# mungerct/Stabilized_Navier_Stokes_Flow_FEniCSx

Hardware: NVIDIA B200
Metric: NS Jacobian+residual assembly throughput (higher is better)
Workload: dtype f64

## Files before the change

### stabilized_navier_stokes_flow_fenicsx_b200/csrc/element_p1tet.cuh

```cuda
#pragma once
#include "element_generic.cuh"

namespace nsgpu {

#if defined(__CUDA_ARCH__)
#define NS_RSQRT(x) rsqrt(x)
#else
#define NS_RSQRT(x) (1.0 / sqrt(x))
#endif

constexpr double P1T_A = 0.1381966011250105;
constexpr double P1T_E = 0.4472135954999579;

template <bool WANT_J, bool WANT_F>
NS_HD void p1tet_rowslab(const FormParams& fp, const bool row_is_origin, const double (&x)[4][3], const double (&u)[4][3],
                         const double (&p)[4], double (&blk)[4][16], double (&fr)[4]) {
  double J[3][3];
#pragma unroll
  for (int i = 0; i < 3; ++i)
#pragma unroll
    for (int j = 0; j < 3; ++j) J[i][j] = x[j + 1][i] - x[0][i];
  const double c00 = J[1][1] * J[2][2] - J[1][2] * J[2][1];
  const double c01 = J[1][2] * J[2][0] - J[1][0] * J[2][2];
  const double c02 = J[1][0] * J[2][1] - J[1][1] * J[2][0];
// ... 229 lines not shown
      s[i] += wt * pt.uq[i];
      Y3[i] += be * pt.Gu[i];
      if (WANT_F) sup[i] += al * pt.uq[i];
    }
    {
      const double w0 = wt * pt.uq[0], w1 = wt * pt.uq[1], w2 = wt * pt.uq[2];
      Q[0] += w0 * pt.uq[0]; Q[1] += w0 * pt.uq[1]; Q[2] += w0 * pt.uq[2];
      Q[3] += w1 * pt.uq[1]; Q[4] += w1 * pt.uq[2]; Q[5] += w2 * pt.uq[2];
    }
    if (WANT_J) {
#pragma unroll
      for (int d = 0; d < 3; ++d) {
        const double bg = be * pt.Gu[d];
#pragma unroll
        for (int c = 0; c < 3; ++c) Y1[d][c] += bg * pt.uq[c];
      }
    }
    if (q == 0) {
      pt0 = pt;
#pragma unroll
      for (int d = 0; d < 3; ++d) ub[d] = W * (P1T_A * U[d] + P1T_E * pt.uq[d]);
    } else if (WANT_J) {
      scratch.put(q, pt);
    }
  }
  nuLbar *= itrG;

  const double TR0 = tbar * Pg0 + H[0] * s[0] + H[1] * s[1] + H[2] * s[2];
  scratch.get_D(D);

  if (WANT_F) {
    const double pbarV = W * (p[0] + p[1] + p[2] + p[3]);
#pragma unroll
    for (int c = 0; c < 3; ++c)
      fr[c] = D[c][0] * ub[0] + D[c][1] * ub[1] + D[c][2] * ub[2] + fp.nu * V * H[c] - pbarV * g[0][c] + sup[c] + nuLbar * divu * g[0][c];
    fr[3] = W * divu + TR0;
  }

  if (WANT_J) {
    const double kap = divu * itrG;
    const double M_off = W * (4.0 * P1T_A * P1T_A + 2.0 * P1T_A * P1T_E);
    const double akap = P1T_A * kap;
    const double ZG[3] = {G[0] * s[0] + G[1] * s[1] + G[2] * s[2], G[1] * s[0] + G[3] * s[1] + G[4] * s[2],
                          G[2] * s[0] + G[4] * s[1] + G[5] * s[2]};
    double C0[3][3], P0[3];
#pragma unroll
    for (int c = 0; c < 3; ++c)
#pragma unroll
      for (int d = 0; d < 3; ++d)
        C0[c][d] = M_off * D[c][d] + P1T_A * (s[c] * H[d] - Y1[d][c]) + akap * ZG[d] * g[0][c];
#pragma unroll
    for (int d = 0; d < 3; ++d) P0[d] = P1T_A * (tbar * H[d] - Y3[d]);
    const double dia0 = P1T_A * TR0;
    const double nuV = fp.nu * V;
    const double Qm[3][3] = {{Q[0], Q[1], Q[2]}, {Q[1], Q[3], Q[4]}, {Q[2], Q[4], Q[5]}};
#pragma unroll
    for (int n = 0; n < 4; ++n) {
      P1TetPoint pt;
      if (n == 0) pt = pt0; else { scratch.get(n, pt); scratch.get_g(n, g[n]); }
      const double L = g[0][0] * g[n][0] + g[0][1] * g[n][1] + g[0][2] * g[n][2];
      double t1[3], t2[3];
      const double ewk = pt.ew * kap;
#pragma unroll
      for (int d = 0; d < 3; ++d) {
        t1[d] = pt.ew * H[d] - pt.eb * pt.Gu[d];
        t2[d] = ewk * pt.Gu[d] + nuLbar * g[n][d];
      }
      const double dia = ub[0] * g[n][0] + ub[1] * g[n][1] + ub[2] * g[n][2] + nuV * L + dia0 + pt.ea;
      double blk[16];
#pragma unroll
      for (int c = 0; c < 3; ++c) {
#pragma unroll
        for (int d = 0; d < 3; ++d) {
          double v = C0[c][d] + L * Qm[c][d] + pt.uq[c] * t1[d] + g[0][c] * t2[d];
          if (n == 0) v += (W * P1T_E * P1T_E) * D[c][d];
          if (c == d) v += dia;
          blk[4 * c + d] = v;
        }
        blk[4 * c + 3] = s[c] * L - W * g[0][c];
      }
#pragma unroll
      for (int d = 0; d < 3; ++d) blk[12 + d] = P0[d] + W * g[n][d] + t1[d] + s[d] * L;
      blk[15] = tbar * L;
      emit(n, blk);
    }
  }
}

}
struct nsgpu_ctx;
namespace nsgpu {
bool p1tet_fast_available(nsgpu_ctx* ctx);
int p1tet_assemble(nsgpu_ctx* ctx, const double* d_xin, bool want_J, bool want_F, double* d_Fout, int part = 0, int sm_reserve = 0);
bool p1tet_can_split(nsgpu_ctx* ctx);
int p1tet_build_plan(nsgpu_ctx* ctx);
void p1tet_free(nsgpu_ctx* ctx);
void p1tet_mark_bc_dirty(nsgpu_ctx* ctx);
int p1tet_spmv(nsgpu_ctx* ctx, const double* d_x, double* d_y);
struct P1BlockView { int64_t n_ent; const int64_t* pair0; const int32_t* ns; const int64_t* rowpos; const int32_t* rowdof; };
bool p1tet_block_view(nsgpu_ctx* ctx, P1BlockView* out);
int p1tet_assemble_streamed(nsgpu_ctx* ctx, const double* x_host, double* F_host);
}
```

### stabilized_navier_stokes_flow_fenicsx_b200/csrc/p1tet.cu

```cuda
#include <algorithm>
#include <cstdio>
#include <vector>
#include <cstdlib>
#include <cub/cub.cuh>

#include "common.cuh"
#include "element_p1tet.cuh"

constexpr int TILE_MAX_ENT = 40;
constexpr int PIPE_VCAP = 128;

struct TileHdr {
  int64_t e0;
  int64_t boff;
  int nent, ninc, nslots, nv;
};

struct nsgpu_p1tet_plan {
  int64_t n_inc = 0, n_ent = 0, n_tiles = 0, n_slots = 0;
  int cap = 0, maxdeg = 0, max_nent = 0;
  uint32_t* d_inc_cell = nullptr;
  int4* d_inc_vtx = nullptr;
  int4* d_inc_lead = nullptr;
  int2* d_tile_vlist = nullptr;
// ... 252 lines not shown
        int pick = pos;
        if (want >= 0)
          for (int c = pos; c < len[l]; ++c)
            if (((base[l] + (lst[l][c] >> 2)) & 7) == want) { pick = c; break; }
        const uint8_t tmp = lst[l][pos]; lst[l][pos] = lst[l][pick]; lst[l][pick] = tmp;
      }
    }
  }
  (void)nt;
}

__global__ void __launch_bounds__(128) k_tile_vlist(TileHdr* __restrict__ hdr, const int4* __restrict__ p_vtx, const int4* __restrict__ p_lead,
                                                    int2* __restrict__ vlist, uint32_t* __restrict__ inc_loc, int* max_nv) {
  using Sort = cub::BlockRadixSort<uint32_t, 128, 4>;
  using Scan = cub::BlockScan<int, 128>;
  __shared__ union { typename Sort::TempStorage sort; typename Scan::TempStorage scan; } tmp;
  __shared__ uint32_t sorted[512], uniq[512];
  const int64_t t = blockIdx.x;
  const int tid = threadIdx.x;
  const int ninc = hdr[t].ninc;
  const int4 vt = p_vtx[t * 128 + tid], ld = p_lead[t * 128 + tid];
  const uint32_t vtx[4] = {(uint32_t)vt.x, (uint32_t)vt.y, (uint32_t)vt.z, (uint32_t)vt.w};
  const int lead[4] = {ld.x, ld.y, ld.z, ld.w};
  uint32_t keys[4];
#pragma unroll
  for (int a = 0; a < 4; ++a) keys[a] = tid < ninc ? vtx[a] : 0xffffffffu;
  Sort(tmp.sort).Sort(keys);
#pragma unroll
  for (int k = 0; k < 4; ++k) sorted[4 * tid + k] = keys[k];
  __syncthreads();
  int flags[4], pos[4], total = 0;
#pragma unroll
  for (int k = 0; k < 4; ++k) {
    const int i = 4 * tid + k;
    flags[k] = (keys[k] != 0xffffffffu && (i == 0 || sorted[i - 1] != keys[k])) ? 1 : 0;
  }
  Scan(tmp.scan).ExclusiveSum(flags, pos, total);
#pragma unroll
  for (int k = 0; k < 4; ++k)
    if (flags[k]) uniq[pos[k]] = keys[k];
  __syncthreads();
  uint32_t packed = 0;
  if (tid < ninc) {
#pragma unroll
    for (int a = 0; a < 4; ++a) {
      int lo = 0, hi = total - 1;
      while (lo < hi) {
        const int mid = (lo + hi) >> 1;
        if (uniq[mid] < vtx[a]) lo = mid + 1; else hi = mid;
      }
      if (lo < PIPE_VCAP) vlist[t * PIPE_VCAP + lo] = make_int2((int)vtx[a], lead[a]);
      packed |= (uint32_t)(lo & 255) << (8 * a);
    }
  }
  __shared__ uint32_t first_packed;
  if (tid == 0) first_packed = packed;
  __syncthreads();
  inc_loc[t * 128 + tid] = tid < ninc ? packed : first_packed;
  if (tid == 0) { hdr[t].nv = total; atomicMax(max_nv, total); }
}

constexpr uint32_t INC_BC_BIT = 0x80000000u;
__global__ void k_inc_bc(int64_t n, uint32_t* __restrict__ inc_cell, const int32_t* __restrict__ dofmap, const uint8_t* __restrict__ marker) {
  const int64_t i = blockIdx.x * (int64_t)blockDim.x + threadIdx.x;
  if (i >= n) return;
  const uint32_t cm = inc_cell[i] & ~INC_BC_BIT;
  const int64_t c = cm >> 2;
  uint8_t f = 0;
  if (marker)
    for (int k = 0; k < 16; ++k) f |= marker[dofmap[c * 16 + k]];
  inc_cell[i] = cm | (f ? INC_BC_BIT : 0u);
}

template <int CAP, int ECAP = CAP> struct TileSmem {
  static constexpr int kBytes = ((5 * CAP + 1 + 15) & ~15) + ((4 * CAP + 15) & ~15) + ((CAP + 15) & ~15);
  static constexpr size_t stageJ = 16 * (size_t)CAP * sizeof(double4);
  static constexpr size_t stageF = (size_t)CAP * sizeof(double4);
  static constexpr size_t tables = 32 * ECAP + 16 * ECAP + 8 * (ECAP + 2) + 4 * CAP + kBytes;
  static constexpr size_t bytes(bool want_J) { return (want_J ? stageJ : 0) + stageF + tables; }
};

template <int CAP_, bool WANT_J, int ECAP = CAP_> struct TileView {
  static constexpr int CAP = CAP_;
  double2* stageJ; double4* stageF; int64_t* rowpos; int4* rowdof; int2* rel; uint32_t* src; uint8_t* bytes;
  __device__ explicit TileView(unsigned char* raw) {
    stageJ = reinterpret_cast<double2*>(raw);
    stageF = reinterpret_cast<double4*>(stageJ + (WANT_J ? 32 * CAP : 0));
    rowpos = reinterpret_cast<int64_t*>(stageF + CAP);
    rowdof = reinterpret_cast<int4*>(rowpos + 4 * ECAP);
    rel = reinterpret_cast<int2*>(rowdof + ECAP);
    src = reinterpret_cast<uint32_t*>(rel + (ECAP + 2));
    bytes = reinterpret_cast<uint8_t*>(src + CAP);
  }
};

__device__ __forceinline__ void cp_async16(void* smem, const void* gmem) {
  asm volatile("cp.async.cg.shared.global [%0], [%1], 16;\n" ::"r"((unsigned)__cvta_generic_to_shared(smem)), "l"(gmem) : "memory");
}
__device__ __forceinline__ void cp_async16_ca(void* smem, const void* gmem) {
  asm volatile("cp.async.ca.shared.global [%0], [%1], 16;\n" ::"r"((unsigned)__cvta_generic_to_shared(smem)), "l"(gmem) : "memory");
}
__device__ __forceinline__ void cp_async8(void* smem, const void* gmem) {
  asm volatile("cp.async.ca.shared.global [%0], [%1], 8;\n" ::"r"((unsigned)__cvta_generic_to_shared(smem)), "l"(gmem) : "memory");
}
__device__ __forceinline__ void cp_async4(void* smem, const void* gmem) {
  asm volatile("cp.async.ca.shared.global [%0], [%1], 4;\n" ::"r"((unsigned)__cvta_generic_to_shared(smem)), "l"(gmem) : "memory");
}
__device__ __forceinline__ void cp_async_commit() { asm volatile("cp.async.commit_group;\n" ::: "memory"); }
__device__ __forceinline__ void cp_async_wait_all() { asm volatile("cp.async.wait_all;\n" ::: "memory"); }
template <int N> __device__ __forceinline__ void cp_async_wait_group() { asm volatile("cp.async.wait_group %0;\n" ::"n"(N) : "memory"); }

template <int CAP, int NT, bool WANT_J, class View>
__device__ __forceinline__ void tile_tables_async(const View& v, const TileHdr& h, int tid, int64_t tile,
                                                  const uint32_t* __restrict__ src, const uint8_t* __restrict__ tile_bytes,
                                                  const int2* __restrict__ ent_rel, const int64_t* __restrict__ rowpos,
                                                  const int4* __restrict__ rowdof) {
  if (WANT_J) {
    for (int k = tid; k < CAP / 4; k += NT) cp_async16(v.src + 4 * k, src + tile * CAP + 4 * k);
    const int nb = (pad16(h.nslots + h.nent + 1) + pad16(h.nslots) + pad16(h.nent)) >> 4;
    for (int k = tid; k < nb; k += NT) cp_async16(v.bytes + 16 * k, tile_bytes + h.boff + 16 * k);
  }
  for (int k = tid; k < h.nent; k += NT) {
    cp_async8(v.rel + k, ent_rel + h.e0 + k);
    cp_async16(v.rowdof + k, rowdof + h.e0 + k);
    if (WANT_J) {
      cp_async16(v.rowpos + 4 * k, rowpos + 4 * (h.e0 + k));
      cp_async16(v.rowpos + 4 * k + 2, rowpos + 4 * (h.e0 + k) + 2);
    }
  }
  if (tid == 0) v.rel[h.nent] = make_int2(h.ninc, h.nslots);
}

__device__ __forceinline__ double quad_sum_b(double v) {
  v += __shfl_xor_sync(0xffffffffu, v, 1);
  v += __shfl_xor_sync(0xffffffffu, v, 2);
  return v;
}

__device__ __forceinline__ int stage_idx(const int CAP, const int n, const int k, const int i) { return (n * 8 + k) * CAP + i; }

__device__ __forceinline__ void store_piece(double* dst, const double4& a, const bool wide) {
  if (wide) {
    asm volatile("st.global.cs.v4.f64 [%0], {%1, %2, %3, %4};" ::"l"(dst), "d"(a.x), "d"(a.y), "d"(a.z), "d"(a.w) : "memory");
  } else {
    __stcs(reinterpret_cast<double2*>(dst), make_double2(a.x, a.y));
    __stcs(reinterpret_cast<double2*>(dst) + 1, make_double2(a.z, a.w));
  }
}

template <int CAP, int NT, bool WANT_J, bool WANT_F, class View>
__device__ __forceinline__ void tile_gather(const View& v, const TileHdr& h, int tid, double* __restrict__ vals,
                                            double* __restrict__ F, const bool wide = false) {
  const uint8_t* s_ss = v.bytes;
  const uint8_t* eos = v.bytes + pad16(h.nslots + h.nent + 1);
  const uint8_t* dg = eos + pad16(h.nslots);
  if (WANT_J) {
    const uint8_t* srcb = reinterpret_cast<const uint8_t*>(v.src);
    for (int ls = tid; ls < h.nslots; ls += NT) {
      const int le = eos[ls];
      const int2 rel = v.rel[le];
      const int s = ls - rel.y;
      if (s == dg[le]) continue;
      const uint8_t* ss = s_ss + ls + le;
      const int jb = ss[0], je = ss[1];
      const uint8_t* sp = srcb + 4 * rel.x;
      double4 acc[4];
// ... 4 lines not shown
#pragma unroll
        for (int i = 0; i < 3; ++i) {
          const bool ok = q + i < je;
          const int code = ok ? sp[q + i] : 0;
          const double2* blkp = v.stageJ + (code & 3) * 8 * CAP + rel.x + (code >> 2);
#pragma unroll
          for (int k = 0; k < 8; ++k) t[i][k] = ok ? blkp[k * CAP] : make_double2(0.0, 0.0);
        }
#pragma unroll
        for (int r = 0; r < 4; ++r) {
          acc[r].x += (t[0][2 * r].x + t[1][2 * r].x) + t[2][2 * r].x;
          acc[r].y += (t[0][2 * r].y + t[1][2 * r].y) + t[2][2 * r].y;
          acc[r].z += (t[0][2 * r + 1].x + t[1][2 * r + 1].x) + t[2][2 * r + 1].x;
          acc[r].w += (t[0][2 * r + 1].y + t[1][2 * r + 1].y) + t[2][2 * r + 1].y;
        }
      }
#pragma unroll
      for (int r = 0; r < 4; ++r) {
        double* dst = vals + v.rowpos[4 * le + r] + 4 * s;
        store_piece(dst, acc[r], wide);
      }
    }
  }
  {
    const int nD = 16 * h.nent;
    const double* sf = reinterpret_cast<const double*>(v.stageF);
    for (int base = 0; base < nD; base += NT) {
      const int item = base + (NT - 1 - tid);
      const int part = item & 3, r = (item >> 2) & 3, le = item >> 4;
      double4 acc = make_double4(0.0, 0.0, 0.0, 0.0);
      double accF = 0.0;
      if (le < h.nent) {
        const int ib = v.rel[le].x, ie = v.rel[le + 1].x;
        for (int ii = ib + part; ii < ie; ii += 12) {
          double2 lo[3], hi[3];
          double f[3];
#pragma unroll
          for (int i = 0; i < 3; ++i) {
            const int i2 = ii + 4 * i;
            const bool ok = i2 < ie;
            if (WANT_J) {
              lo[i] = ok ? v.stageJ[(2 * r) * CAP + i2] : make_double2(0.0, 0.0);
              hi[i] = ok ? v.stageJ[(2 * r + 1) * CAP + i2] : make_double2(0.0, 0.0);
            }
            if (WANT_F) f[i] = ok ? sf[4 * i2 + r] : 0.0;
          }
          if (WANT_J) {
            acc.x += (lo[0].x + lo[1].x) + lo[2].x; acc.y += (lo[0].y + lo[1].y) + lo[2].y;
            acc.z += (hi[0].x + hi[1].x) + hi[2].x; acc.w += (hi[0].y + hi[1].y) + hi[2].y;
          }
          if (WANT_F) accF += (f[0] + f[1]) + f[2];
        }
      }
      if (WANT_J) { acc.x = quad_sum_b(acc.x); acc.y = quad_sum_b(acc.y); acc.z = quad_sum_b(acc.z); acc.w = quad_sum_b(acc.w); }
      if (WANT_F) accF = quad_sum_b(accF);
      if (le < h.nent && part == 0) {
        if (WANT_J) {
          double* dst = vals + v.rowpos[4 * le + r] + 4 * dg[le];
          store_piece(dst, acc, wide);
        }
        if (WANT_F) {
          const int4 rd = v.rowdof[le];
          F[(r == 0) ? rd.x : (r == 1) ? rd.y : (r == 2) ? rd.z : rd.w] = accF;
        }
      }
    }
  }
}

#define P1_KERNEL_ARGS                                                                                                     \
  FormParams form, const double *__restrict__ xg, const double *__restrict__ wv, const int32_t *__restrict__ members,          \
      const bool contiguous, const uint8_t *__restrict__ bc_marker, const double *__restrict__ bc_value,                        \
      const uint32_t *__restrict__ inc_cell, const int4 *__restrict__ inc_vtx,                                                  \
      const int4 *__restrict__ inc_lead, const uint32_t *__restrict__ src, const uint8_t *__restrict__ tile_bytes,               \
      const int2 *__restrict__ ent_rel, const int64_t *__restrict__ rowpos, const int4 *__restrict__ rowdof,                     \
      const TileHdr *__restrict__ tile_hdr, double *__restrict__ vals, double *__restrict__ F, const int64_t n_tiles

#define P1_PHASE_ARGS                                                                                                      \
  const FormParams &form, const double *__restrict__ xg, const double *__restrict__ wv, const int32_t *__restrict__ members,  \
      const bool contiguous, const uint8_t *__restrict__ bc_marker, const double *__restrict__ bc_value

struct NoHook { __device__ __forceinline__ void operator()() const {} };

template <int CAP, bool WANT_J, bool WANT_F, class View, class Hook = NoHook>
__device__ __forceinline__ void phase_a_core(const View& v, const int tid, const int (&lead)[4], const uint32_t cm, const double (&x)[4][3],
                                             const double (&u)[4][3], const double (&p)[4], P1_PHASE_ARGS, Hook before_first_write = Hook()) {
  {
    const bool has_bc = (cm & INC_BC_BIT) != 0;
    double fr[4] = {0.0, 0.0, 0.0, 0.0};
    const bool row_is_origin = (cm & 3u) == 0;
    bool rowbc[4] = {false, false, false, false};
    if (has_bc) {
#pragma unroll
      for (int r = 0; r < 4; ++r) rowbc[r] = bc_marker[contiguous ? lead[0] + r : members[(int64_t)lead[0] * KMAX + r]] != 0;
    }
    auto emit = [&](const int n, double (&blk)[16]) {
      if (has_bc) {
#pragma unroll
        for (int d = 0; d < 4; ++d) {
          const int32_t dj = contiguous ? lead[n] + d : members[(int64_t)lead[n] * KMAX + d];
          if (bc_marker[dj]) {
            const double delta = bc_value[dj] - wv[dj];
#pragma unroll
            for (int r = 0; r < 4; ++r) {
              if (WANT_F) fr[r] += blk[4 * r + d] * delta;
              blk[4 * r + d] = 0.0;
            }
          }
        }
#pragma unroll
        for (int r = 0; r < 4; ++r)
          if (rowbc[r]) {
#pragma unroll
            for (int d = 0; d < 4; ++d) blk[4 * r + d] = 0.0;
          }
      }
      if (WANT_J) {
#pragma unroll
        for (int r = 0; r < 4; ++r)
        {
          v.stageJ[stage_idx(CAP, n, 2 * r, tid)] = make_double2(blk[4 * r], blk[4 * r + 1]);
          v.stageJ[stage_idx(CAP, n, 2 * r + 1, tid)] = make_double2(blk[4 * r + 2], blk[4 * r + 3]);
        }
      }
    };
    if (WANT_J) {
      struct SmemScratch {
        double2* st;
        int tid;
        Hook& hook;
        __device__ double after_geometry(double w) const { return w; }
        __device__ void put_geom(const double (&g)[4][3], const double (&D)[3][3]) const {
          hook();
#ifndef NS_NO_PARK
          sts2(stage_idx(CAP, 0, 0, tid), D[0][0], D[0][1]); sts2(stage_idx(CAP, 0, 1, tid), D[0][2], D[1][0]);
          sts2(stage_idx(CAP, 0, 2, tid), D[1][1], D[1][2]); sts2(stage_idx(CAP, 0, 3, tid), D[2][0], D[2][1]);
#ifndef NS_PARK_D_ONLY
          sts2(stage_idx(CAP, 0, 4, tid), D[2][2], g[1][2]); sts2(stage_idx(CAP, 0, 5, tid), g[2][2], g[3][2]);
#pragma unroll
          for (int n = 1; n < 4; ++n) sts2(stage_idx(CAP, n, 5, tid), g[n][0], g[n][1]);
#else
          sts2(stage_idx(CAP, 0, 4, tid), D[2][2], 0.0);
          (void)g;
#endif
#endif
        }
        __device__ void get_D(double (&D)[3][3]) const {
#ifndef NS_NO_PARK
          double t;
          lds2(stage_idx(CAP, 0, 0, tid), D[0][0], D[0][1]); lds2(stage_idx(CAP, 0, 1, tid), D[0][2], D[1][0]);
          lds2(stage_idx(CAP, 0, 2, tid), D[1][1], D[1][2]); lds2(stage_idx(CAP, 0, 3, tid), D[2][0], D[2][1]);
          lds2(stage_idx(CAP, 0, 4, tid), D[2][2], t);
#ifndef NS_PARK_D_ONLY
          double g2, g3;
          lds2(stage_idx(CAP, 0, 5, tid), g2, g3);
          sts2(stage_idx(CAP, 1, 6, tid), t, 0.0); sts2(stage_idx(CAP, 2, 6, tid), g2, 0.0); sts2(stage_idx(CAP, 3, 6, tid), g3, 0.0);
#endif
#endif
        }
        __device__ void get_g(int n, double (&gn)[3]) const {
#if !defined(NS_NO_PARK) && !defined(NS_PARK_D_ONLY)
          double pad;
          lds2(stage_idx(CAP, n, 5, tid), gn[0], gn[1]);
          lds2(stage_idx(CAP, n, 6, tid), gn[2], pad);
#else
          (void)n; (void)gn;
#endif
        }
        __device__ void sts2(int idx, double a, double b) const {
          asm volatile("st.shared.v2.f64 [%0], {%1, %2};" ::"r"((unsigned)__cvta_generic_to_shared(st + idx)), "d"(a), "d"(b) : "memory");
        }
        __device__ void lds2(int idx, double& a, double& b) const {
          asm volatile("ld.shared.v2.f64 {%0, %1}, [%2];" : "=d"(a), "=d"(b) : "r"((unsigned)__cvta_generic_to_shared(st + idx)) : "memory");
        }
        __device__ void put(int q, const P1TetPoint& pt) const {
          st[stage_idx(CAP, q, 0, tid)] = make_double2(pt.uq[0], pt.uq[1]); st[stage_idx(CAP, q, 1, tid)] = make_double2(pt.uq[2], pt.Gu[0]);
          st[stage_idx(CAP, q, 2, tid)] = make_double2(pt.Gu[1], pt.Gu[2]); st[stage_idx(CAP, q, 3, tid)] = make_double2(pt.ew, pt.eb);
          st[stage_idx(CAP, q, 4, tid)] = make_double2(pt.ea, 0.0);
        }
        __device__ void get(int q, P1TetPoint& pt) const {
          const double2 a = st[stage_idx(CAP, q, 0, tid)], b = st[stage_idx(CAP, q, 1, tid)], c = st[stage_idx(CAP, q, 2, tid)],
                        d = st[stage_idx(CAP, q, 3, tid)], e = st[stage_idx(CAP, q, 4, tid)];
          pt.uq[0] = a.x; pt.uq[1] = a.y; pt.uq[2] = b.x; pt.Gu[0] = b.y;
          pt.Gu[1] = c.x; pt.Gu[2] = c.y; pt.ew = d.x; pt.eb = d.y; pt.ea = e.x;
        }
      } scratch{v.stageJ, tid, before_first_write};
      p1tet_rowslab2<true, WANT_F>(form, row_is_origin, x, u, p, fr, scratch, emit);
    } else {
      struct LocalScratch {
        P1TetPoint q[4];
        __device__ double after_geometry(double w) const { return w; }
        __device__ void put_geom(const double (&)[4][3], const double (&)[3][3]) const {}
        __device__ void get_D(double (&)[3][3]) const {}
        __device__ void get_g(int, double (&)[3]) const {}
        __device__ void put(int i, const P1TetPoint& pt) { q[i] = pt; }
        __device__ void get(int i, P1TetPoint& pt) const { pt = q[i]; }
      } scratch;
      before_first_write();
      if (has_bc) p1tet_rowslab2<true, WANT_F>(form, row_is_origin, x, u, p, fr, scratch, emit);
      else p1tet_rowslab2<false, WANT_F>(form, row_is_origin, x, u, p, fr, scratch, emit);
    }
    if (WANT_F) v.stageF[tid] = make_double4(fr[0], fr[1], fr[2], fr[3]);
  }
}

template <int CAP, bool WANT_J, bool WANT_F, class View>
__device__ __forceinline__ void phase_a(const View& v, const int tid, const int4 vt, const int4 ld, const uint32_t cm, P1_PHASE_ARGS) {
  const int vtx[4] = {vt.x, vt.y, vt.z, vt.w};
  const int lead[4] = {ld.x, ld.y, ld.z, ld.w};
  double x[4][3], u[4][3], p[4];
#pragma unroll
  for (int a = 0; a < 4; ++a) {
    const double* xp = xg + 3 * (int64_t)vtx[a];
    x[a][0] = xp[0]; x[a][1] = xp[1]; x[a][2] = xp[2];
    if (contiguous) {
      const double2* wp = reinterpret_cast<const double2*>(wv + lead[a]);
      const double2 w01 = wp[0], w23 = wp[1];
      u[a][0] = w01.x; u[a][1] = w01.y; u[a][2] = w23.x; p[a] = w23.y;
    } else {
      const int4 mem = reinterpret_cast<const int4*>(members)[lead[a]];
      u[a][0] = wv[mem.x]; u[a][1] = wv[mem.y]; u[a][2] = wv[mem.z]; p[a] = wv[mem.w];
    }
  }
  phase_a_core<CAP, WANT_J, WANT_F>(v, tid, lead, cm, x, u, p, form, xg, wv, members, contiguous, bc_marker, bc_value);
}

template <int CAP, int MINB, bool WANT_J, bool WANT_F>
__global__ void __launch_bounds__(CAP, MINB) k_p1tet_tiles(P1_KERNEL_ARGS) {
  extern __shared__ __align__(16) unsigned char smem_raw[];
  const TileView<CAP, WANT_J> v(smem_raw);
  const int tid = threadIdx.x;
  for (int64_t tile = blockIdx.x; tile < n_tiles; tile += gridDim.x) {
    const int4 vt = inc_vtx[tile * CAP + tid];
    const int4 ld = inc_lead[tile * CAP + tid];
    const uint32_t cm = inc_cell[tile * CAP + tid];
    const TileHdr h = tile_hdr[tile];
    {
      const int64_t nt = tile + gridDim.x;
      if (nt < n_tiles) {
        asm volatile("prefetch.global.L1 [%0];" ::"l"(inc_vtx + nt * CAP + tid));
        asm volatile("prefetch.global.L1 [%0];" ::"l"(inc_lead + nt * CAP + tid));
        if ((tid & 7) == 0) asm volatile("prefetch.global.L1 [%0];" ::"l"(inc_cell + nt * CAP + tid));
        if (tid == 0) asm volatile("prefetch.global.L2 [%0];" ::"l"(tile_hdr + nt));
        if (WANT_J && (tid & 7) == 0) asm volatile("prefetch.global.L2 [%0];" ::"l"(src + nt * CAP + tid));
      }
    }
    if (h.nent <= 0) continue;
    tile_tables_async<CAP, CAP, WANT_J>(v, h, tid, tile, src, tile_bytes, ent_rel, rowpos, rowdof);
    if (tid < h.ninc) phase_a<CAP, WANT_J, WANT_F>(v, tid, vt, ld, cm, form, xg, wv, members, contiguous, bc_marker, bc_value);
    cp_async_wait_all();
    __syncthreads();
    tile_gather<CAP, CAP, WANT_J, WANT_F>(v, h, tid, vals, F);
    __syncthreads();
  }
}

constexpr int PIPE_ECAP = TILE_MAX_ENT;
constexpr int PIPE_VREC = 5;
template <bool WANT_J> struct PipeSmem {
  static constexpr int CAP = 128;
  static constexpr size_t view = TileSmem<CAP, PIPE_ECAP>::bytes(WANT_J);
  static constexpr size_t table = (size_t)PIPE_VCAP * PIPE_VREC * sizeof(double2);
  static constexpr size_t ring = PIPE_VCAP * sizeof(int2) + 2 * CAP * sizeof(uint32_t);
  static constexpr size_t bytes = view + 2 * table + 3 * ring + 3 * sizeof(TileHdr);
};

template <bool WANT_J, bool WANT_F>
__global__ void __launch_bounds__(128, 2) k_p1tet_pipe(P1_KERNEL_ARGS, const int2* __restrict__ tile_vlist, const uint32_t* __restrict__ inc_loc,
                                                       const int64_t tile0, const bool wide) {
  constexpr int CAP = 128;
  using View = TileView<CAP, WANT_J, PIPE_ECAP>;
  using PS = PipeSmem<WANT_J>;
  extern __shared__ __align__(16) unsigned char smem_raw[];
  const View v(smem_raw);
  double2* tab = reinterpret_cast<double2*>(smem_raw + PS::view);
  unsigned char* ring = smem_raw + PS::view + 2 * PS::table;
  TileHdr* r_hdr = reinterpret_cast<TileHdr*>(ring + 3 * PS::ring);
  const int tid = threadIdx.x;
  const int nj = (int)((n_tiles - (int64_t)blockIdx.x + gridDim.x - 1) / gridDim.x);
// ... 708 lines not shown
```

### stabilized_navier_stokes_flow_fenicsx_b200/csrc/p1tet_ws.cuh

```cuda
#pragma once

namespace nsgpu {

constexpr int WS_SS = 120;
constexpr int WS_VCAP = 96;
constexpr int WS_NBUF = 3;
#ifndef WS_REG_COMPUTE
#define WS_REG_COMPUTE 208
#define WS_REG_GATHER 48
#endif
constexpr int WS_CBLOB = 8 * WS_VCAP + 512 + 512 + 16;
constexpr int WS_LIST = 8;
constexpr int WS_OVF = 256;
constexpr int WS_HMAX = 32 + 16 * TILE_MAX_ENT + 32 * WS_VCAP + 2 * WS_OVF;
static_assert(WS_HMAX % 16 == 0 && WS_CBLOB % 16 == 0, "bulk copies move multiples of 16 bytes");

struct WsHdr { int nent, ninc, n_off, pad0; int64_t vbase; int64_t pad1; };
struct WsVrec { uint16_t ib, ie; uint32_t diag_off; uint32_t rowlen; int32_t dof0; };
struct WsSrec { uint16_t len, ovf; uint32_t out_off; uint32_t rowlen; uint32_t pad; uint16_t list[WS_LIST]; };

template <bool WANT_J> struct WsSmem {
  static constexpr size_t stage = (WANT_J ? (size_t)32 * WS_SS * sizeof(double2) : 0) + (size_t)WS_SS * sizeof(double4);
  static constexpr size_t vtab = (size_t)WS_VCAP * PIPE_VREC * sizeof(double2);
  static constexpr size_t off_htab = WS_NBUF * stage;
// ... 149 lines not shown
        for (int b = 0; b < 8; ++b) parent_lane_of_bank[b] = -1;
        queue[qt++] = l;
        while (qh < qt && !found) {
          const int cur = queue[qh++];
          for (int b = 0; b < 8 && !found; ++b) {
            if (!((cand[cur] >> b) & 1u) || ((visited >> b) & 1u)) continue;
            visited |= 1u << b;
            parent_lane_of_bank[b] = cur;
            if (owner[b] < 0) { found = true; end_bank = b; }
            else if (qt < 8) queue[qt++] = owner[b];
          }
        }
        if (found) {
          int b = end_bank;
          while (b >= 0) {
            const int ln = parent_lane_of_bank[b];
            int nb = -1;
            for (int k = 0; k < 8; ++k) if (owner[k] == ln) nb = k;
            owner[b] = ln;
            if (ln == l) break;
            b = nb;
          }
        }
      }
      for (int l = 0; l < 8; ++l) {
        if (pos >= len[l]) continue;
        int want = -1;
        for (int b = 0; b < 8; ++b) if (owner[b] == l) want = b;
        int pick = pos;
        if (want >= 0)
          for (int c = pos; c < len[l]; ++c)
            if ((lst[l][c] & 7) == want) { pick = c; break; }
        const uint16_t tmpv = lst[l][pos]; lst[l][pos] = lst[l][pick]; lst[l][pick] = tmpv;
      }
    }
  }
}

__device__ __forceinline__ int ws_src_lane(int k, int ninc) { return k < WS_SS ? k : (k - 8 < ninc ? k - 8 : k); }

__global__ void __launch_bounds__(128) k_ws_cblob(const TileHdr* __restrict__ hdr, const int2* __restrict__ vlist, const uint32_t* __restrict__ inc_loc,
                                                  uint8_t* __restrict__ cblob) {
  const int64_t t = blockIdx.x;
  const int tid = threadIdx.x;
  const TileHdr h = hdr[t];
  uint8_t* C = cblob + t * WS_CBLOB;
  if (tid < WS_VCAP) reinterpret_cast<int2*>(C)[tid] = tid < h.nv ? vlist[t * PIPE_VCAP + tid] : make_int2(0, 0);
  const int src = ws_src_lane(tid, h.ninc);
  reinterpret_cast<uint32_t*>(C + 8 * WS_VCAP)[tid] = inc_loc[t * 128 + src];
  if (tid == 0) *reinterpret_cast<int4*>(C + 8 * WS_VCAP + 1024) = make_int4(h.nv, h.ninc, 0, 0);
}

__global__ void k_ws_cm(int64_t n, const TileHdr* __restrict__ hdr, const uint32_t* __restrict__ inc_cell, uint8_t* __restrict__ cblob) {
  const int64_t i = blockIdx.x * (int64_t)blockDim.x + threadIdx.x;
  if (i >= n) return;
  const int64_t t = i >> 7;
  const int k = (int)(i & 127);
  const int ninc = hdr[t].ninc;
  const int src = ws_src_lane(k, ninc);
  reinterpret_cast<uint32_t*>(cblob + t * WS_CBLOB + 8 * WS_VCAP + 512)[k] = src < ninc ? inc_cell[t * 128 + src] : 0u;
}

__device__ __forceinline__ uint32_t smem_u32(const void* p) { return (uint32_t)__cvta_generic_to_shared(p); }
__device__ __forceinline__ void named_bar_sync(int id, int count) { asm volatile("bar.sync %0, %1;" ::"r"(id), "r"(count) : "memory"); }
__device__ __forceinline__ void named_bar_arrive(int id, int count) { asm volatile("bar.arrive %0, %1;" ::"r"(id), "r"(count) : "memory"); }
__device__ __forceinline__ void mbar_init(uint64_t* b, int count) {
  asm volatile("mbarrier.init.shared::cta.b64 [%0], %1;" ::"r"(smem_u32(b)), "r"(count) : "memory");
}
__device__ __forceinline__ void mbar_expect_tx(uint64_t* b, uint32_t bytes) {
  asm volatile("mbarrier.arrive.expect_tx.shared::cta.b64 _, [%0], %1;" ::"r"(smem_u32(b)), "r"(bytes) : "memory");
}
__device__ __forceinline__ void bulk_g2s(void* dst, const void* src, uint32_t bytes, uint64_t* b) {
  asm volatile("cp.async.bulk.shared::cluster.global.mbarrier::complete_tx::bytes [%0], [%1], %2, [%3];" ::"r"(smem_u32(dst)), "l"(src), "r"(bytes),
               "r"(smem_u32(b))
               : "memory");
}
__device__ __forceinline__ void mbar_wait(uint64_t* b, uint32_t parity) {
  uint32_t ok;
  do {
    asm volatile("{\n .reg .pred p;\n mbarrier.try_wait.parity.shared::cta.b64 p, [%1], %2;\n selp.u32 %0, 1, 0, p;\n}" : "=r"(ok) : "r"(smem_u32(b)), "r"(parity) : "memory");
  } while (!ok);
}

struct WsView { double2* stageJ; double4* stageF; };

template <bool WANT_J, bool WANT_F>
__device__ __forceinline__ void ws_gather(const unsigned char* __restrict__ H, const double2* __restrict__ stageJ, const double4* __restrict__ stageF,
                                          const int tid, double* __restrict__ vals, double* __restrict__ F, const bool wide) {
  const int4 hd = *reinterpret_cast<const int4*>(H);
  const int64_t vbase = *reinterpret_cast<const int64_t*>(H + 16);
  const int nent = hd.x, n_off = hd.z;
  const int lane = tid & 31, warp = tid >> 5;
  const int n_grp = WANT_J ? (n_off + 7) >> 3 : 0;
  const int r = lane >> 3;
  const double2* base = stageJ + 2 * r * WS_SS;
  for (int item = warp; item < n_grp + nent; item += 4) {
    if (item < n_grp) {
      const int j = 8 * item + (lane & 7);
      if (j < n_off) {
        const unsigned char* rec = H + 32 + 16 * nent + 32 * j;
        const int4 sr = *reinterpret_cast<const int4*>(rec);
        const uint4 lw = *reinterpret_cast<const uint4*>(rec + 16);
        const int len = sr.x & 0xffff, n0 = len < WS_LIST ? len : WS_LIST;
        double4 acc = make_double4(0.0, 0.0, 0.0, 0.0);
#pragma unroll
        for (int q2 = 0; q2 < WS_LIST / 2; ++q2) {
          if (2 * q2 < n0) {
            const uint32_t w = q2 == 0 ? lw.x : (q2 == 1 ? lw.y : (q2 == 2 ? lw.z : lw.w));
            const uint32_t i0 = w & 0xffffu;
            const double2 a0 = base[i0], a1 = base[i0 + WS_SS];
            acc.x += a0.x; acc.y += a0.y; acc.z += a1.x; acc.w += a1.y;
            if (2 * q2 + 1 < n0) {
              const double2 b0 = base[w >> 16], b1 = base[(w >> 16) + WS_SS];
              acc.x += b0.x; acc.y += b0.y; acc.z += b1.x; acc.w += b1.y;
            }
          }
        }
        if (len > WS_LIST) {
          const uint16_t* ov = reinterpret_cast<const uint16_t*>(H + 32 + 16 * nent + 32 * n_off) + ((unsigned)sr.x >> 16);
          for (int q = WS_LIST; q < len; ++q) {
            const double2 a0 = base[ov[q - WS_LIST]], a1 = base[ov[q - WS_LIST] + WS_SS];
            acc.x += a0.x; acc.y += a0.y; acc.z += a1.x; acc.w += a1.y;
          }
        }
        store_piece(vals + vbase + (uint32_t)sr.y + (int64_t)r * (uint32_t)sr.z, acc, wide);
      }
    } else {
      const int le = item - n_grp, part = lane & 7;
      const int4 vr = *reinterpret_cast<const int4*>(H + 32 + 16 * le);
      const int ib = vr.x & 0xffff, ie = (unsigned)vr.x >> 16;
      const double* sf = reinterpret_cast<const double*>(stageF);
      double4 acc = make_double4(0.0, 0.0, 0.0, 0.0);
      double accF = 0.0;
#pragma unroll 2
      for (int i = ib + part; i < ie; i += 8) {
        if (WANT_J) {
          const double2 a0 = base[i], a1 = base[WS_SS + i];
          acc.x += a0.x; acc.y += a0.y; acc.z += a1.x; acc.w += a1.y;
        }
        if (WANT_F) accF += sf[4 * i + r];
      }
#pragma unroll
      for (int o = 1; o < 8; o <<= 1) {
        if (WANT_J) {
          acc.x += __shfl_xor_sync(0xffffffffu, acc.x, o); acc.y += __shfl_xor_sync(0xffffffffu, acc.y, o);
          acc.z += __shfl_xor_sync(0xffffffffu, acc.z, o); acc.w += __shfl_xor_sync(0xffffffffu, acc.w, o);
        }
        if (WANT_F) accF += __shfl_xor_sync(0xffffffffu, accF, o);
      }
      if (part == 0) {
        if (WANT_J) store_piece(vals + vbase + (uint32_t)vr.y + (int64_t)r * (uint32_t)vr.z, acc, wide);
        if (WANT_F) F[vr.w + r] = accF;
      }
    }
  }
}

template <bool WANT_J, bool WANT_F>
__global__ void __launch_bounds__(512, 1)
k_p1tet_ws(const FormParams form, const double* __restrict__ xg, const double* __restrict__ wv, const uint8_t* __restrict__ bc_marker,
           const double* __restrict__ bc_value, const uint8_t* __restrict__ cblob, const uint8_t* __restrict__ hblob, const uint64_t* __restrict__ hword,
           double* __restrict__ vals, double* __restrict__ F, const int64_t n_tiles, const int64_t tile0, const bool wide) {
  using S = WsSmem<WANT_J>;
  extern __shared__ __align__(16) unsigned char smem_raw[];
  const int wg = threadIdx.x >> 7;
  const int tid = threadIdx.x & 127;
  const int nk = (int)((n_tiles - (int64_t)blockIdx.x + gridDim.x - 1) / gridDim.x);
  uint64_t* bars = reinterpret_cast<uint64_t*>(smem_raw + S::off_bar);
  if (threadIdx.x == 0) {
    for (int i = 0; i < 7; ++i) mbar_init(bars + i, 1);
    asm volatile("fence.mbarrier_init.release.cluster;" ::: "memory");
  }
  __syncthreads();
  auto stage_of = [&](int b) { return smem_raw + (size_t)b * S::stage; };
  if (wg < 2) {
    asm volatile("setmaxnreg.inc.sync.aligned.u32 %0;" ::"n"(WS_REG_COMPUTE));
    const int g = wg;
    const int nm = nk > g ? (nk - g + 1) / 2 : 0;
    unsigned char* ring = smem_raw + S::off_ring + (size_t)g * 2 * WS_CBLOB;
    double2* tab = reinterpret_cast<double2*>(smem_raw + S::off_vtab + (size_t)g * S::vtab);
    uint64_t* rbar = bars + 3 + 2 * g;
    auto fetch_ring = [&](const int m) {
      const int64_t t = tile0 + (int64_t)blockIdx.x + (int64_t)(g + 2 * m) * gridDim.x;
      mbar_expect_tx(rbar + (m & 1), WS_CBLOB);
      bulk_g2s(ring + (m & 1) * WS_CBLOB, cblob + t * WS_CBLOB, WS_CBLOB, rbar + (m & 1));
    };
    auto fetch_table = [&](const int m) {
      const unsigned char* rs = ring + (m & 1) * WS_CBLOB;
      const int n = *reinterpret_cast<const int*>(rs + 8 * WS_VCAP + 1024) * PIPE_VREC;
      const int2* vl = reinterpret_cast<const int2*>(rs);
      for (int item = tid; item < n; item += 128) {
        const int i = item / PIPE_VREC, c = item - i * PIPE_VREC;
        const int2 e = vl[i];
        if (c < 3) cp_async8(reinterpret_cast<double*>(tab + i * PIPE_VREC) + c, xg + 3 * (int64_t)e.x + c);
        else cp_async16_ca(tab + i * PIPE_VREC + (c - 1), wv + e.y + 2 * (c - 3));
      }
    };
    if (nm > 0) {
      if (tid == 0) { fetch_ring(0); if (nm > 1) fetch_ring(1); }
      mbar_wait(rbar, 0);
      fetch_table(0);
    }
    cp_async_commit();
    for (int m = 0; m < nm; ++m) {
      const int k = g + 2 * m, b = k % 3;
      cp_async_wait_all();
      named_bar_sync(7 + g, 128);
      const unsigned char* rs = ring + (m & 1) * WS_CBLOB;
      const uint32_t loc = reinterpret_cast<const uint32_t*>(rs + 8 * WS_VCAP)[tid];
      const uint32_t cm = reinterpret_cast<const uint32_t*>(rs + 8 * WS_VCAP + 512)[tid];
      const int ninc = reinterpret_cast<const int*>(rs + 8 * WS_VCAP + 1024)[1];
      double x[4][3], u[4][3], p[4];
      int lead[4] = {0, 0, 0, 0};
#pragma unroll
      for (int a = 0; a < 4; ++a) {
        const int i = (loc >> (8 * a)) & 255;
        const double2* rec = tab + i * PIPE_VREC;
        const double2 q0 = rec[0], q1 = rec[1], q2 = rec[2], q3 = rec[3];
        x[a][0] = q0.x; x[a][1] = q0.y; x[a][2] = q1.x;
        u[a][0] = q2.x; u[a][1] = q2.y; u[a][2] = q3.x; p[a] = q3.y;
        if (cm & INC_BC_BIT) lead[a] = reinterpret_cast<const int2*>(rs)[i].y;
      }
      named_bar_sync(7 + g, 128);
      if (m + 1 < nm) {
        mbar_wait(rbar + ((m + 1) & 1), ((m + 1) >> 1) & 1);
        fetch_table(m + 1);
      }
      cp_async_commit();
      if (tid == 0 && m + 2 < nm) fetch_ring(m + 2);
      const WsView v{reinterpret_cast<double2*>(stage_of(b)), reinterpret_cast<double4*>(stage_of(b) + (WANT_J ? (size_t)32 * WS_SS * sizeof(double2) : 0))};
      auto wait_empty = [&]() { if (k >= WS_NBUF) named_bar_sync(4 + b, 256); };
      const int col = tid < WS_SS ? tid : tid - 8;
      if ((tid & ~31) < ninc)
        phase_a_core<WS_SS, WANT_J, WANT_F>(v, col, lead, cm, x, u, p, form, xg, wv, nullptr, true, bc_marker, bc_value, wait_empty);
      else
        wait_empty();
      __threadfence_block();
      named_bar_arrive(1 + b, 256);
    }
  } else {
    asm volatile("setmaxnreg.dec.sync.aligned.u32 %0;" ::"n"(WS_REG_GATHER));
    const int h = wg - 2;
    unsigned char* htab = smem_raw + S::off_htab;
    auto word_of = [&](const int k) { return hword[tile0 + (int64_t)blockIdx.x + (int64_t)k * gridDim.x]; };
    auto fetch_h = [&](const int k, const uint64_t w) {
      const int b = k % WS_NBUF;
      const uint32_t bytes = (uint32_t)(w & 0xffff) << 4;
      mbar_expect_tx(bars + b, bytes);
      bulk_g2s(htab + (size_t)b * WS_HMAX, hblob + ((w >> 16) << 4), bytes, bars + b);
    };
    uint64_t wnext = 0;
    if (tid == 0) {
      if (h == 0) for (int k = 0; k < nk && k < WS_NBUF; ++k) fetch_h(k, word_of(k));
      if (h + WS_NBUF < nk) wnext = word_of(h + WS_NBUF);
    }
    for (int j = h; j < nk; j += 2) {
      const int b = j % WS_NBUF;
      mbar_wait(bars + b, (j / WS_NBUF) & 1);
      named_bar_sync(1 + b, 256);
      const unsigned char* st = stage_of(b);
      ws_gather<WANT_J, WANT_F>(htab + (size_t)b * WS_HMAX, reinterpret_cast<const double2*>(st),
                                reinterpret_cast<const double4*>(st + (WANT_J ? (size_t)32 * WS_SS * sizeof(double2) : 0)), tid, vals, F, wide);
      if (j + WS_NBUF < nk) {
        named_bar_sync(9 + h, 128);
        named_bar_arrive(4 + b, 256);
        if (tid == 0) {
          fetch_h(j + WS_NBUF, wnext);
          if (j + 2 + WS_NBUF < nk) wnext = word_of(j + 2 + WS_NBUF);
        }
      }
    }
  }
}

}
```

Before: 2122.

## Park per-element scratch in Blackwell tensor memory instead of shared memory

In the warp-specialized kernel, the compute warpgroups now keep the parked geometry (D matrix, basis gradients) and per-quadrature-point values in TMEM. They use tcgen05.st/ld instead of shared-memory staging or registers, and allocate 256 TMEM columns per CTA with a named barrier so deallocation waits until all warps finish. The goal is to cut shared-memory traffic and register pressure in the Jacobian path, freeing shared bandwidth for the gather stage. In exchange it adds synchronous TMEM load waits, alloc/dealloc overhead, and a hook call moved to the first emit. Some leftover NS_NO_PARK ifdef variants are also removed.

```diff
diff --git a/stabilized_navier_stokes_flow_fenicsx_b200/csrc/element_p1tet.cuh b/stabilized_navier_stokes_flow_fenicsx_b200/csrc/element_p1tet.cuh
--- a/stabilized_navier_stokes_flow_fenicsx_b200/csrc/element_p1tet.cuh
+++ b/stabilized_navier_stokes_flow_fenicsx_b200/csrc/element_p1tet.cuh
@@ -335,6 +335,7 @@
 #pragma unroll
       for (int d = 0; d < 3; ++d) blk[12 + d] = P0[d] + W * g[n][d] + t1[d] + s[d] * L;
       blk[15] = tbar * L;
+      if (n == 0) scratch.before_first_emit();
       emit(n, blk);
     }
   }
diff --git a/stabilized_navier_stokes_flow_fenicsx_b200/csrc/p1tet.cu b/stabilized_navier_stokes_flow_fenicsx_b200/csrc/p1tet.cu
--- a/stabilized_navier_stokes_flow_fenicsx_b200/csrc/p1tet.cu
+++ b/stabilized_navier_stokes_flow_fenicsx_b200/csrc/p1tet.cu
@@ -358,6 +358,7 @@
 
 template <int CAP_, bool WANT_J, int ECAP = CAP_> struct TileView {
   static constexpr int CAP = CAP_;
+  static constexpr bool tmem_scratch = false;
   double2* stageJ; double4* stageF; int64_t* rowpos; int4* rowdof; int2* rel; uint32_t* src; uint8_t* bytes;
   __device__ explicit TileView(unsigned char* raw) {
     stageJ = reinterpret_cast<double2*>(raw);
@@ -528,6 +529,48 @@
 
 struct NoHook { __device__ __forceinline__ void operator()() const {} };
 
+#define NS_TM_LH(v) "r"(__double2loint(v)), "r"(__double2hiint(v))
+__device__ __forceinline__ void tmem_st1(uint32_t a, double x0) {
+  asm volatile("tcgen05.st.sync.aligned.32x32b.x2.b32 [%0], {%1, %2};" ::"r"(a), NS_TM_LH(x0) : "memory");
+}
+__device__ __forceinline__ void tmem_st2(uint32_t a, double x0, double x1) {
+  asm volatile("tcgen05.st.sync.aligned.32x32b.x4.b32 [%0], {%1, %2, %3, %4};" ::"r"(a), NS_TM_LH(x0), NS_TM_LH(x1) : "memory");
+}
+__device__ __forceinline__ void tmem_st8(uint32_t a, const double (&x)[8]) {
+  asm volatile("tcgen05.st.sync.aligned.32x32b.x16.b32 [%0], {%1, %2, %3, %4, %5, %6, %7, %8, %9, %10, %11, %12, %13, %14, %15, %16};" ::"r"(a),
+               NS_TM_LH(x[0]), NS_TM_LH(x[1]), NS_TM_LH(x[2]), NS_TM_LH(x[3]), NS_TM_LH(x[4]), NS_TM_LH(x[5]), NS_TM_LH(x[6]), NS_TM_LH(x[7])
+               : "memory");
+}
+__device__ __forceinline__ void tmem_st16(uint32_t a, const double (&x)[16]) {
+  asm volatile("tcgen05.st.sync.aligned.32x32b.x32.b32 [%0], {%1, %2, %3, %4, %5, %6, %7, %8, %9, %10, %11, %12, %13, %14, %15, %16, "
+               "%17, %18, %19, %20, %21, %22, %23, %24, %25, %26, %27, %28, %29, %30, %31, %32};" ::"r"(a),
+               NS_TM_LH(x[0]), NS_TM_LH(x[1]), NS_TM_LH(x[2]), NS_TM_LH(x[3]), NS_TM_LH(x[4]), NS_TM_LH(x[5]), NS_TM_LH(x[6]), NS_TM_LH(x[7]),
+               NS_TM_LH(x[8]), NS_TM_LH(x[9]), NS_TM_LH(x[10]), NS_TM_LH(x[11]), NS_TM_LH(x[12]), NS_TM_LH(x[13]), NS_TM_LH(x[14]), NS_TM_LH(x[15])
+               : "memory");
+}
+#undef NS_TM_LH
+__device__ __forceinline__ void tmem_ld1(uint32_t a, double& x0) {
+  uint32_t r[2];
+  asm volatile("tcgen05.ld.sync.aligned.32x32b.x2.b32 {%0, %1}, [%2];\n\ttcgen05.wait::ld.sync.aligned;" : "=r"(r[0]), "=r"(r[1]) : "r"(a) : "memory");
+  x0 = __hiloint2double(r[1], r[0]);
+}
+__device__ __forceinline__ void tmem_ld2(uint32_t a, double& x0, double& x1) {
+  uint32_t r[4];
+  asm volatile("tcgen05.ld.sync.aligned.32x32b.x4.b32 {%0, %1, %2, %3}, [%4];\n\ttcgen05.wait::ld.sync.aligned;"
+               : "=r"(r[0]), "=r"(r[1]), "=r"(r[2]), "=r"(r[3]) : "r"(a) : "memory");
+  x0 = __hiloint2double(r[1], r[0]); x1 = __hiloint2double(r[3], r[2]);
+}
+__device__ __forceinline__ void tmem_ld8(uint32_t a, double (&x)[8]) {
+  uint32_t r[16];
+  asm volatile("tcgen05.ld.sync.aligned.32x32b.x16.b32 {%0, %1, %2, %3, %4, %5, %6, %7, %8, %9, %10, %11, %12, %13, %14, %15}, [%16];\n\t"
+               "tcgen05.wait::ld.sync.aligned;"
+               : "=r"(r[0]), "=r"(r[1]), "=r"(r[2]), "=r"(r[3]), "=r"(r[4]), "=r"(r[5]), "=r"(r[6]), "=r"(r[7]), "=r"(r[8]), "=r"(r[9]),
+                 "=r"(r[10]), "=r"(r[11]), "=r"(r[12]), "=r"(r[13]), "=r"(r[14]), "=r"(r[15])
+               : "r"(a) : "memory");
+#pragma unroll
+  for (int i = 0; i < 8; ++i) x[i] = __hiloint2double(r[2 * i + 1], r[2 * i]);
+}
+
 template <int CAP, bool WANT_J, bool WANT_F, class View, class Hook = NoHook>
 __device__ __forceinline__ void phase_a_core(const View& v, const int tid, const int (&lead)[4], const uint32_t cm, const double (&x)[4][3],
                                              const double (&u)[4][3], const double (&p)[4], P1_PHASE_ARGS, Hook before_first_write = Hook()) {
@@ -570,7 +613,44 @@
         }
       }
     };
-    if (WANT_J) {
+    if constexpr (WANT_J && View::tmem_scratch) {
+      struct TmemScratch {
+        uint32_t a;
+        Hook& hook;
+        __device__ double after_geometry(double w) const { return w; }
+        __device__ void put_geom(const double (&g)[4][3], const double (&D)[3][3]) const {
+          const double x[16] = {D[0][0], D[0][1], D[0][2], D[1][0], D[1][1], D[1][2], D[2][0], D[2][1],
+                                D[2][2], g[1][0], g[1][1], g[1][2], g[2][0], g[2][1], g[2][2], g[3][0]};
+          tmem_st16(a, x);
+          tmem_st2(a + 32, g[3][1], g[3][2]);
+        }
+        __device__ void get_D(double (&D)[3][3]) const {
+          asm volatile("tcgen05.wait::st.sync.aligned;" ::: "memory");
+          double x[8];
+          tmem_ld8(a, x);
+          D[0][0] = x[0]; D[0][1] = x[1]; D[0][2] = x[2]; D[1][0] = x[3]; D[1][1] = x[4]; D[1][2] = x[5]; D[2][0] = x[6]; D[2][1] = x[7];
+          tmem_ld1(a + 16, D[2][2]);
+        }
+        __device__ void get_g(int n, double (&gn)[3]) const {
+          const uint32_t c = a + 18 + 6 * (n - 1);
+          if (n & 1) { tmem_ld1(c, gn[0]); tmem_ld2(c + 2, gn[1], gn[2]); }
+          else { tmem_ld2(c, gn[0], gn[1]); tmem_ld1(c + 4, gn[2]); }
+        }
+        __device__ void put(int q, const P1TetPoint& pt) const {
+          const double x[8] = {pt.uq[0], pt.uq[1], pt.uq[2], pt.Gu[0], pt.Gu[1], pt.Gu[2], pt.ew, pt.eb};
+          tmem_st8(a + 32 + 16 * q, x);
+          tmem_st1(a + 94 + 2 * q, pt.ea);
+        }
+        __device__ void get(int q, P1TetPoint& pt) const {
+          double x[8];
+          tmem_ld8(a + 32 + 16 * q, x);
+          pt.uq[0] = x[0]; pt.uq[1] = x[1]; pt.uq[2] = x[2]; pt.Gu[0] = x[3]; pt.Gu[1] = x[4]; pt.Gu[2] = x[5]; pt.ew = x[6]; pt.eb = x[7];
+          tmem_ld1(a + 94 + 2 * q, pt.ea);
+        }
+        __device__ void before_first_emit() const { hook(); }
+      } scratch{v.tmem, before_first_write};
+      p1tet_rowslab2<true, WANT_F>(form, row_is_origin, x, u, p, fr, scratch, emit);
+    } else if constexpr (WANT_J) {
       struct SmemScratch {
         double2* st;
         int tid;
@@ -578,41 +658,27 @@
         __device__ double after_geometry(double w) const { return w; }
         __device__ void put_geom(const double (&g)[4][3], const double (&D)[3][3]) const {
           hook();
-#ifndef NS_NO_PARK
           sts2(stage_idx(CAP, 0, 0, tid), D[0][0], D[0][1]); sts2(stage_idx(CAP, 0, 1, tid), D[0][2], D[1][0]);
           sts2(stage_idx(CAP, 0, 2, tid), D[1][1], D[1][2]); sts2(stage_idx(CAP, 0, 3, tid), D[2][0], D[2][1]);
-#ifndef NS_PARK_D_ONLY
           sts2(stage_idx(CAP, 0, 4, tid), D[2][2], g[1][2]); sts2(stage_idx(CAP, 0, 5, tid), g[2][2], g[3][2]);
 #pragma unroll
           for (int n = 1; n < 4; ++n) sts2(stage_idx(CAP, n, 5, tid), g[n][0], g[n][1]);
-#else
-          sts2(stage_idx(CAP, 0, 4, tid), D[2][2], 0.0);
-          (void)g;
-#endif
-#endif
         }
         __device__ void get_D(double (&D)[3][3]) const {
-#ifndef NS_NO_PARK
           double t;
           lds2(stage_idx(CAP, 0, 0, tid), D[0][0], D[0][1]); lds2(stage_idx(CAP, 0, 1, tid), D[0][2], D[1][0]);
           lds2(stage_idx(CAP, 0, 2, tid), D[1][1], D[1][2]); lds2(stage_idx(CAP, 0, 3, tid), D[2][0], D[2][1]);
           lds2(stage_idx(CAP, 0, 4, tid), D[2][2], t);
-#ifndef NS_PARK_D_ONLY
           double g2, g3;
           lds2(stage_idx(CAP, 0, 5, tid), g2, g3);
           sts2(stage_idx(CAP, 1, 6, tid), t, 0.0); sts2(stage_idx(CAP, 2, 6, tid), g2, 0.0); sts2(stage_idx(CAP, 3, 6, tid), g3, 0.0);
-#endif
-#endif
         }
         __device__ void get_g(int n, double (&gn)[3]) const {
-#if !defined(NS_NO_PARK) && !defined(NS_PARK_D_ONLY)
           double pad;
           lds2(stage_idx(CAP, n, 5, tid), gn[0], gn[1]);
           lds2(stage_idx(CAP, n, 6, tid), gn[2], pad);
-#else
-          (void)n; (void)gn;
-#endif
-        }
+        }
+        __device__ void before_first_emit() const {}
         __device__ void sts2(int idx, double a, double b) const {
           asm volatile("st.shared.v2.f64 [%0], {%1, %2};" ::"r"((unsigned)__cvta_generic_to_shared(st + idx)), "d"(a), "d"(b) : "memory");
         }
@@ -641,6 +707,7 @@
         __device__ void get_g(int, double (&)[3]) const {}
         __device__ void put(int i, const P1TetPoint& pt) { q[i] = pt; }
         __device__ void get(int i, P1TetPoint& pt) const { pt = q[i]; }
+        __device__ void before_first_emit() const {}
       } scratch;
       before_first_write();
       if (has_bc) p1tet_rowslab2<true, WANT_F>(form, row_is_origin, x, u, p, fr, scratch, emit);
diff --git a/stabilized_navier_stokes_flow_fenicsx_b200/csrc/p1tet_ws.cuh b/stabilized_navier_stokes_flow_fenicsx_b200/csrc/p1tet_ws.cuh
--- a/stabilized_navier_stokes_flow_fenicsx_b200/csrc/p1tet_ws.cuh
+++ b/stabilized_navier_stokes_flow_fenicsx_b200/csrc/p1tet_ws.cuh
@@ -255,7 +255,14 @@
   } while (!ok);
 }
 
-struct WsView { double2* stageJ; double4* stageF; };
+constexpr int WS_TMEM_COLS = 256;
+__device__ __forceinline__ void tmem_fence_before() { asm volatile("tcgen05.fence::before_thread_sync;" ::: "memory"); }
+__device__ __forceinline__ void tmem_fence_after() { asm volatile("tcgen05.fence::after_thread_sync;" ::: "memory"); }
+
+struct WsView {
+  static constexpr bool tmem_scratch = true;
+  double2* stageJ; double4* stageF; uint32_t tmem;
+};
 
 template <bool WANT_J, bool WANT_F>
 __device__ __forceinline__ void ws_gather(const unsigned char* __restrict__ H, const double2* __restrict__ stageJ, const double4* __restrict__ stageF,
@@ -340,11 +347,17 @@
   const int tid = threadIdx.x & 127;
   const int nk = (int)((n_tiles - (int64_t)blockIdx.x + gridDim.x - 1) / gridDim.x);
   uint64_t* bars = reinterpret_cast<uint64_t*>(smem_raw + S::off_bar);
+  const uint32_t tmem_slot = smem_u32(smem_raw) + (uint32_t)(S::off_bar + 7 * sizeof(uint64_t));
+  auto tmem_base = [&]() { uint32_t a; asm volatile("ld.shared.u32 %0, [%1];" : "=r"(a) : "r"(tmem_slot) : "memory"); return a; };
+  if (threadIdx.x < 32)
+    asm volatile("tcgen05.alloc.cta_group::1.sync.aligned.shared::cta.b32 [%0], %1;" ::"r"(tmem_slot), "n"(WS_TMEM_COLS) : "memory");
   if (threadIdx.x == 0) {
     for (int i = 0; i < 7; ++i) mbar_init(bars + i, 1);
     asm volatile("fence.mbarrier_init.release.cluster;" ::: "memory");
   }
+  tmem_fence_before();
   __syncthreads();
+  tmem_fence_after();
   auto stage_of = [&](int b) { return smem_raw + (size_t)b * S::stage; };
   if (wg < 2) {
     asm volatile("setmaxnreg.inc.sync.aligned.u32 %0;" ::"n"(WS_REG_COMPUTE));
@@ -401,7 +414,8 @@
       }
       cp_async_commit();
       if (tid == 0 && m + 2 < nm) fetch_ring(m + 2);
-      const WsView v{reinterpret_cast<double2*>(stage_of(b)), reinterpret_cast<double4*>(stage_of(b) + (WANT_J ? (size_t)32 * WS_SS * sizeof(double2) : 0))};
+      const WsView v{reinterpret_cast<double2*>(stage_of(b)), reinterpret_cast<double4*>(stage_of(b) + (WANT_J ? (size_t)32 * WS_SS * sizeof(double2) : 0)),
+                     tmem_base() + ((uint32_t)(tid & 96) << 16) + 128u * g};
       auto wait_empty = [&]() { if (k >= WS_NBUF) named_bar_sync(4 + b, 256); };
       const int col = tid < WS_SS ? tid : tid - 8;
       if ((tid & ~31) < ninc)
@@ -411,8 +425,16 @@
       __threadfence_block();
       named_bar_arrive(1 + b, 256);
     }
+    tmem_fence_before();
+    named_bar_sync(11, 512);
+    if (threadIdx.x < 32) {
+      tmem_fence_after();
+      asm volatile("tcgen05.dealloc.cta_group::1.sync.aligned.b32 %0, %1;" ::"r"(tmem_base()), "n"(WS_TMEM_COLS) : "memory");
+      asm volatile("tcgen05.relinquish_alloc_permit.cta_group::1.sync.aligned;" ::: "memory");
+    }
   } else {
     asm volatile("setmaxnreg.dec.sync.aligned.u32 %0;" ::"n"(WS_REG_GATHER));
+    named_bar_arrive(11, 512);
     const int h = wg - 2;
     unsigned char* htab = smem_raw + S::off_htab;
     auto word_of = [&](const int k) { return hword[tile0 + (int64_t)blockIdx.x + (int64_t)k * gridDim.x]; };
```

New measurement: 2227, median of 6. 1.05x the previous value.
